# alex880317/LeGO-LOAM-SR

Measured on AMD Instinct MI355X. Metric: scans/sec (VLP-16 1800x16) at 1/2/4/8 GPUs; pose delta vs CPU ref, higher is better.
Workload: dtype fp32; 1 GPU; configs[1]: VLP-16 1800x16 projection + ground/cluster segmentation + curvature/feature extraction, labels/indices bit-exact vs CPU; lidar=VLP-16, rings=16, columns=1800, distinct_clouds_per_gpu=16, streams_per_gpu=3, parallelism=scan-sharded x1

## Files before the change

### lego-loam-sr_amd/csrc/llsr_fa.hip

```cpp
#include <cfloat>
#include <climits>

#include "llsr_device.h"
#include "llsr_imu.h"
#include "llsr_isort.h"
#include "llsr_libm.h"

namespace llsr {

using namespace llsr_libm;
constexpr double kPi = 3.14159265358979323846;

constexpr int kFaT = 256;
constexpr int kFaTile = 4 * kFaT - 12;

__device__ __forceinline__ float4 loam_point_rel(const DevCfg& c, float4 p, int i, int first, float start, float endo,
                                                 float diff, float* rel) {
  float o = -atan2f_(p.y, p.x);
  if (i <= first) {
    o = ori_branch1(o, start);
  } else {
    o = (float)(o + 2 * kPi);
    if ((double)o < (double)endo - kPi * 3 / 2) o = (float)(o + 2 * kPi);
    else if ((double)o > (double)endo + kPi / 2) o = (float)(o - 2 * kPi);
// ... 317 lines not shown
  const int l = lane_id();
  const unsigned long long lt = (1ull << l) - 1ull;
  int nsel = 0;
  for (int t0 = 0; t0 < nc; t0 += 64) {
    const int t = t0 + l;
    const bool valid = t < nc;
    const int ind = valid ? order(t) : 0;
    const int w = valid ? ind - ws : 0;
    const int r = valid ? wflag[w] : 0x80;
    bool alive = valid && (r & 0x80) == 0;
    const int lo = w - ((r >> 3) & 7), hi = w + (r & 7);
    unsigned long long sel = 0ull;
    unsigned long long m = __ballot(alive);
    while (m) {
      const int s = __ffsll((long long)m) - 1;
      const int slo = __builtin_amdgcn_readlane(lo, s), shi = __builtin_amdgcn_readlane(hi, s);
      sel |= 1ull << s;
      if (l > s && w >= slo && w <= shi) alive = false;
      if (l == s) alive = false;
      m = __ballot(alive);
    }
    if ((sel >> l) & 1ull) {
      wlab[w] = lab;
      outp[nsel + __popcll(sel & lt)] = ind;
      for (int q = lo; q <= hi; ++q) wflag[q] = (uint8_t)(wflag[q] | 0x80);
    }
    nsel += __popcll(sel);
    __builtin_amdgcn_fence(__ATOMIC_SEQ_CST, "wavefront");
    __builtin_amdgcn_wave_barrier();
  }
  return nsel;
}

__global__ __launch_bounds__(256, 5) void k_select_ring(DevCfg c, DevBufs d) {
  __shared__ uint64_t key[kRingMax];
  __shared__ uint32_t win_raw[2 * kWin / 4];
  uint8_t* wflag = reinterpret_cast<uint8_t*>(win_raw);
  int8_t* wlab = reinterpret_cast<int8_t*>(wflag + kWin);
  __shared__ uint16_t cfirst[kWin / 64 + 1];
  __shared__ uint16_t cpos[kRingMax];
  __shared__ uint16_t rstart[kRingMax + 1];
  __shared__ int tmp[8];
  __shared__ float red[6][4];
  __shared__ int s_cnt;
  const int i = blockIdx.x, b = blockIdx.y;
  const int H = c.H, HW = c.HW;
  const size_t base = (size_t)b * HW;
  const int tid = threadIdx.x, nt = blockDim.x;
  int* rc = d.ring_cnt + (size_t)b * 3 * H;
  const int sp = d.start_ring[b * H + i];
  const int ep = d.end_ring[b * H + i] - 1;
  if (sp >= ep) {
    if (tid == 0) { rc[i] = 0; rc[H + i] = 0; rc[2 * H + i] = 0; }
    return;
  }
  const float* curv = d.curv + base;
  const int ws = sp - 5 > 0 ? sp - 5 : 0;
  const int we = ep + 5 < HW - 1 ? ep + 5 : HW - 1;
  const int wn = we - ws + 1;
  if (c.dbg_phase <= -2) return;
  constexpr int kPer = (kWin + 255) / 256;
  float cvr[kPer];
  uint32_t cl[kPer];
  uint32_t pkm = 0, gdm = 0;
  {
    uint8_t pk[kPer], gd[kPer];
    int8_t lb[kPer];
#pragma unroll
    for (int u = 0; u < kPer; ++u) {
      const int t = tid + u * 256, pos = ws + t;
      cl[u] = 0;
      if (t < wn) {
        pk[u] = d.picked[base + pos];
        gd[u] = d.seg_ground[base + pos];
        lb[u] = d.clabel[base + pos];
        cl[u] = d.seg_col[base + pos];
        cvr[u] = curv[pos];
      }
    }
#pragma unroll
    for (int u = 0; u < kPer; ++u) {
      const int t = tid + u * 256;
      if (t < wn) {
        wlab[t] = lb[u];
        pkm |= (pk[u] != 0 ? 1u : 0u) << u;
        gdm |= (gd[u] != 0 ? 1u : 0u) << u;
        if ((t & 63) == 0) cfirst[t >> 6] = (uint16_t)cl[u];
      }
    }
  }
  if (tid == 0) s_cnt = 0;
  __syncthreads();
  if (c.dbg_phase <= -1) return;
  {
    uint64_t* gbits = reinterpret_cast<uint64_t*>(key);
    const int l = lane_id();
#pragma unroll
    for (int u = 0; u < kPer; ++u) {
      const int t = tid + u * 256;
      const int dn = __shfl_down((int)cl[u], 1, 64);
      const int nx = l < 63 ? dn : (t + 1 < wn ? (int)cfirst[(t + 1) >> 6] : 0);
      const bool stop = t + 1 >= wn || abs(nx - (int)cl[u]) > 10;
      const uint64_t m = __ballot(t < wn && stop);
      if (l == 0 && (t >> 6) <= (wn >> 6)) gbits[t >> 6] = m;
    }
    __syncthreads();
    const int nw = (wn >> 6) + 1;
#pragma unroll
    for (int u = 0; u < kPer; ++u) {
      const int t = tid + u * 256;
      if (t >= wn) break;
      const int k = t >> 6, sh = t & 63;
      uint64_t fw = gbits[k] >> sh;
      if (sh && k + 1 < nw) fw |= gbits[k + 1] << (64 - sh);
      const int f = fw ? min(5, __ffsll((long long)fw) - 1) : 5;
      int bk = 0;
      if (t > 0) {
        const int q = t - 1, kq = q >> 6, s2 = q & 63;
        uint64_t bw = gbits[kq] << (63 - s2);
        if (s2 < 63 && kq > 0) bw |= gbits[kq - 1] >> (s2 + 1);
        bk = min(min(5, t), bw ? (int)__clzll((long long)bw) : 64);
      }
      wflag[t] = (uint8_t)(f | (bk << 3) | (((gdm >> u) & 1u) << 6) | (((pkm >> u) & 1u) << 7));
    }
  }
  __syncthreads();
  const int nRng = ep - sp;
  const int ph = sp == 4 ? d.phantom[b] : 0;
  const bool ph_in = ph >= ws && ph - ws < wn;
  const float ph_curv = ph < 5 ? 0.0f : curv[ph];
  if (sp == 4 && !ph_in && tid == 0) atomicAdd(&d.counts[b * kCnt + C_PHOUT], 1);
  __shared__ BlockSortLds bsl;
  __shared__ int s_flag, s_exact;
  if (tid == 0) s_flag = 0;
  __syncthreads();
  if (sp == 4) {
#pragma unroll
    for (int u = 0; u < kPer; ++u) {
      const int p = ws + tid + u * 256;
      if (p >= 5 && p < ep && cvr[u] == 0.0f) s_flag = 1;
    }
  }
  auto curv_of = [&](int ind) { return ind < 5 ? 0.0f : curv[ind]; };
  auto exact_sort = [&]() {
    for (int t = tid; t < nRng; t += nt) {
      const int p = sp + t;
      const float v = p == 4 ? 0.0f : curv[p];
      const int ind = p == 4 ? ph : p;
      key[t] = ((uint64_t)__float_as_uint(v) << 32) | (uint32_t)ind;
    }
    block_introsort<256>(key, nRng, cpos, rstart, bsl, CurvLess{});
    if (tid == 0) {
      if (sp == 4) d.phantom[b] = (int)(uint32_t)key[0];
      atomicAdd(&d.counts[b * kCnt + C_EXACT], 1);
      s_exact = 1;
    }
    __syncthreads();
  };
  auto compact_sorted = [&](bool descending, auto elig) {
    const int l = lane_id();
    int cnt = 0;
    for (int c0 = 0; c0 < nRng; c0 += 64) {
      const int k = c0 + l;
      const int t = descending ? nRng - 1 - k : k;
      const bool e = k < nRng && elig((int)(uint32_t)key[t]);
      const unsigned long long m = __ballot(e);
      if (e) cpos[cnt + __popcll(m & ((1ull << l) - 1ull))] = (uint16_t)t;
      cnt += __popcll(m);
    }
    return cnt;
  };
  auto edge_elig = [&](int ind) {
    const int w = ind - ws;
    return w >= 0 && w < wn && (wflag[w] & 0xC0) == 0 && curv_of(ind) > c.edge_thr;
  };
  auto flat_elig = [&](int ind) {
    const int w = ind - ws;
    return w >= 0 && w < wn && (wflag[w] & 0xC0) == 0x40 && curv_of(ind) < c.surf_thr;
  };
  auto append = [&](bool edge) {
#pragma unroll
    for (int u = 0; u < kPer; ++u) {
      const int p = ws + tid + u * 256;
      const bool in = p >= sp && p < ep && (p != 4 || ph_in);
      const int ind = p == 4 ? ph : p;
      const float v = p == 4 ? 0.0f : cvr[u];
      const float ve = p == 4 ? ph_curv : cvr[u];
      const int w = in ? ind - ws : 0;
      const int fg = in ? (wflag[w] & 0xC0) : 0x80;
      const bool e = in && (edge ? (fg == 0 && ve > c.edge_thr) : (fg == 0x40 && ve < c.surf_thr));
      const unsigned long long m = __ballot(e);
      int wb = 0;
      if (lane_id() == 0 && m) wb = atomicAdd(&s_cnt, (int)__popcll(m));
      wb = __builtin_amdgcn_readlane(wb, 0);
      if (e) key[wb + __popcll(m & ((1ull << lane_id()) - 1ull))] = ((uint64_t)__float_as_uint(v) << 32) | (uint32_t)ind;
    }
  };
  auto ties = [&](int lo, int hi) {
    for (int t = lo + tid; t + 1 < hi; t += nt)
      if ((uint32_t)(key[t] >> 32) == (uint32_t)(key[t + 1] >> 32)) s_flag = 1;
    __syncthreads();
    return s_flag != 0;
  };
  if (tid == 0) s_exact = 0;
  __syncthreads();
  const bool epE = curv[ep] > c.edge_thr && (wflag[ep - ws] & 0x40) == 0;
  const int e0 = epE ? 1 : 0;
  append(true);
  __syncthreads();
  if (c.dbg_phase <= 0) return;
  int nE = s_cnt;
  int n2 = max(pow2_ceil(nE), 64);
  for (int t = nE + tid; t < n2; t += nt) key[t] = 0ull;
  __syncthreads();
  block4_sort<uint64_t>(key, n2);
  if (c.dbg_phase <= 1) return;
  if (ties(n2 - nE, n2)) {
    exact_sort();
    if (tid < 64) {
      const int cnt = compact_sorted(true, edge_elig);
      auto order = [&](int t) { return t < e0 ? ep : (int)(uint32_t)key[cpos[t - e0]]; };
      const int sel = greedy_wave(order, cnt + e0, ws, wflag, wlab, (int8_t)1, d.edge_tmp + base + sp);
      if (tid == 0) { rc[i] = sel; s_cnt = 0; }
    }
  } else if (tid < 64) {
    auto order = [&](int t) { return t < e0 ? ep : (int)(uint32_t)key[n2 - 1 - (t - e0)]; };
    const int cnt = greedy_wave(order, nE + e0, ws, wflag, wlab, (int8_t)1, d.edge_tmp + base + sp);
    if (tid == 0) { rc[i] = cnt; s_cnt = 0; }
  }
  __syncthreads();
  if (c.dbg_phase <= 2) return;
  const bool epF = curv[ep] < c.surf_thr && (wflag[ep - ws] & 0x40) != 0;
  if (s_exact) {
    if (tid < 64) {
      const int cnt = compact_sorted(false, flat_elig);
      auto order = [&](int t) { return t < cnt ? (int)(uint32_t)key[cpos[t]] : ep; };
      const int sel = greedy_wave(order, cnt + (epF ? 1 : 0), ws, wflag, wlab, (int8_t)-1, d.flat_tmp + base + sp);
      if (tid == 0) rc[H + i] = sel;
    }
  } else {
    append(false);
    __syncthreads();
    const int nF = s_cnt;
    n2 = max(pow2_ceil(nF), 64);
    for (int t = nF + tid; t < n2; t += nt) key[t] = ~0ull;
    __syncthreads();
    block4_sort<uint64_t>(key, n2);
    if (ties(0, nF)) {
      exact_sort();
      if (tid < 64) {
        const int cnt = compact_sorted(false, flat_elig);
        auto order = [&](int t) { return t < cnt ? (int)(uint32_t)key[cpos[t]] : ep; };
        const int sel = greedy_wave(order, cnt + (epF ? 1 : 0), ws, wflag, wlab, (int8_t)-1, d.flat_tmp + base + sp);
        if (tid == 0) rc[H + i] = sel;
      }
    } else if (tid < 64) {
      auto order = [&](int t) { return t < nF ? (int)(uint32_t)key[t] : ep; };
      const int cnt = greedy_wave(order, nF + (epF ? 1 : 0), ws, wflag, wlab, (int8_t)-1, d.flat_tmp + base + sp);
      if (tid == 0) rc[H + i] = cnt;
    }
  }
  __syncthreads();
  if (c.dbg_phase <= 3) return;
  for (int t = tid; t < wn; t += nt) {
    d.picked[base + ws + t] = (uint8_t)(wflag[t] >> 7);
    d.clabel[base + ws + t] = wlab[t];
  }
  const int n = ep - sp + 1;
  const int per = (n + nt - 1) / nt;
  const int k0 = min(tid * per, n), k1 = min(k0 + per, n);
  int mine = 0;
  for (int k = k0; k < k1; ++k) mine += wlab[sp + k - ws] <= 0;
  int L;
  int pos = block_excl_scan(mine, tmp, &L);
  for (int k = k0; k < k1; ++k)
    if (wlab[sp + k - ws] <= 0) cpos[pos++] = (uint16_t)k;
  __syncthreads();
  if (c.dbg_phase <= 4) return;
  const float4* lp = d.loam + base + sp;
  constexpr int kLp = kRingMax / 256;
  float4 lpr[kLp];
  float mn[3] = {FLT_MAX, FLT_MAX, FLT_MAX}, mx[3] = {-FLT_MAX, -FLT_MAX, -FLT_MAX};
#pragma unroll
  for (int u = 0; u < kLp; ++u)
    if (tid + u * 256 < L) lpr[u] = lp[cpos[tid + u * 256]];
#pragma unroll
  for (int u = 0; u < kLp; ++u) {
    if (tid + u * 256 >= L) continue;
    const float4 p = lpr[u];
    mn[0] = fminf(mn[0], p.x); mn[1] = fminf(mn[1], p.y); mn[2] = fminf(mn[2], p.z);
    mx[0] = fmaxf(mx[0], p.x); mx[1] = fmaxf(mx[1], p.y); mx[2] = fmaxf(mx[2], p.z);
  }
  for (int a = 0; a < 3; ++a) { mn[a] = wave_reduce_min(mn[a]); mx[a] = wave_reduce_max(mx[a]); }
  if (lane_id() == 0)
    for (int a = 0; a < 3; ++a) { red[a][tid >> 6] = mn[a]; red[3 + a][tid >> 6] = mx[a]; }
  __syncthreads();
  for (int a = 0; a < 3; ++a) {
    mn[a] = fminf(fminf(red[a][0], red[a][1]), fminf(red[a][2], red[a][3]));
    mx[a] = fmaxf(fmaxf(red[3 + a][0], red[3 + a][1]), fmaxf(red[3 + a][2], red[3 + a][3]));
  }
  const float inv = 1.0f / 0.2f;
  float4* out = d.lflat_tmp + base + sp;
  if (L == 0) {
    if (tid == 0) rc[2 * H + i] = 0;
    return;
  }
  const long long dx = (long long)((mx[0] - mn[0]) * inv) + 1, dy = (long long)((mx[1] - mn[1]) * inv) + 1,
                  dz = (long long)((mx[2] - mn[2]) * inv) + 1;
  if (dx * dy * dz > (long long)INT_MAX) {
    for (int t = tid; t < L; t += nt) out[t] = lp[cpos[t]];
    if (tid == 0) rc[2 * H + i] = L;
    return;
  }
  int minb[3], div[3];
  for (int a = 0; a < 3; ++a) {
    minb[a] = (int)floorf(mn[a] * inv);
    div[a] = (int)floorf(mx[a] * inv) - minb[a] + 1;
  }
  const int mul1 = div[0], mul2 = div[0] * div[1];
  uint32_t* vk = reinterpret_cast<uint32_t*>(key);
  uint32_t vkr[kLp];
#pragma unroll
  for (int u = 0; u < kLp; ++u) {
    const int t = tid + u * 256;
    vkr[u] = 0u;
    if (t >= L) continue;
    const float4 p = lpr[u];
    const int i0 = (int)(floorf(p.x * inv) - (float)minb[0]);
    const int i1 = (int)(floorf(p.y * inv) - (float)minb[1]);
    const int i2 = (int)(floorf(p.z * inv) - (float)minb[2]);
    vkr[u] = (uint32_t)(i0 + i1 * mul1 + i2 * mul2);
    vk[t] = vkr[u];
  }
  __syncthreads();
  __shared__ int scnt[kLp * 4 + 1];
  const int wv = tid >> 6, ln = lane_id();
  const unsigned long long ltm = (1ull << ln) - 1ull;
  int V;
  auto slot_scan = [&]() {
    __syncthreads();
    if (wv == 0) {
      const int v = ln < kLp * 4 ? scnt[ln] : 0;
      const int incl = wave_incl_scan_add(v);
      if (ln < kLp * 4) scnt[ln] = incl - v;
      if (ln == 63) scnt[kLp * 4] = incl;
    }
    __syncthreads();
  };
  auto sort_runs = [&]() {
    unsigned long long mR[kLp];
#pragma unroll
    for (int u = 0; u < kLp; ++u) {
      const int t = u * 256 + tid;
      mR[u] = __ballot(t < L && (t == 0 || vkr[u] != vk[t - 1]));
      if (ln == 0) scnt[u * 4 + wv] = (int)__popcll(mR[u]);
    }
    slot_scan();
    const int R = scnt[kLp * 4];
#pragma unroll
    for (int u = 0; u < kLp; ++u) {
      if (!((mR[u] >> ln) & 1ull)) continue;
      const int t = u * 256 + tid;
      const int ro = scnt[u * 4 + wv] + (int)__popcll(mR[u] & ltm);
      rstart[ro] = (uint16_t)t;
      key[ro] = ((uint64_t)vkr[u] << 32) | (uint32_t)ro;
    }
    if (tid == 0) rstart[R] = (uint16_t)L;
    const int R2 = max(pow2_ceil(R), 64);
    for (int t = R + tid; t < R2; t += nt) key[t] = ~0ull;
    __syncthreads();
    block4_sort<uint64_t>(key, R2);
    return R;
  };
  if (c.exact_vg) {
    if (c.dbg_phase <= 5) return;
    const int R = sort_runs();
    uint16_t* rrank = reinterpret_cast<uint16_t*>(win_raw);
    const unsigned long long lem = ltm | (1ull << ln);
    unsigned long long mH[kLp];
#pragma unroll
    for (int u = 0; u < kLp; ++u) {
      const int t = u * 256 + tid;
      mH[u] = __ballot(t < R && (t == 0 || (key[t] >> 32) != (key[t - 1] >> 32)));
      if (ln == 0) scnt[u * 4 + wv] = (int)__popcll(mH[u]);
    }
    slot_scan();
#pragma unroll
    for (int u = 0; u < kLp; ++u) {
      const int t = u * 256 + tid;
      if (t < R) rrank[(uint32_t)key[t]] = (uint16_t)(scnt[u * 4 + wv] + (int)__popcll(mH[u] & lem) - 1);
    }
    __syncthreads();
    uint32_t* gk = reinterpret_cast<uint32_t*>(d.ccl_a + base) + sp;
    uint16_t* gc = reinterpret_cast<uint16_t*>(d.ccl_b + base) + sp;
    for (int r = tid; r < R; r += nt) {
      const uint32_t rk = (uint32_t)rrank[r] << 11;
      const int qe = rstart[r + 1];
      for (int q = rstart[r]; q < qe; ++q) gk[q] = rk | (uint32_t)q;
    }
    for (int t = tid; t < L; t += nt) gc[t] = cpos[t];
    if (tid == 0) rc[2 * H + i] = -1 - L;
    return;
  } else {
    if (c.dbg_phase <= 5) return;
    const int R = sort_runs();
    if (c.dbg_phase <= 6) return;
    unsigned long long mH[kLp];
#pragma unroll
    for (int u = 0; u < kLp; ++u) {
      const int t = u * 256 + tid;
      const bool head = t < R && (t == 0 || (key[t] >> 32) != (key[t - 1] >> 32));
      mH[u] = __ballot(head);
      if (ln == 0) scnt[u * 4 + wv] = (int)__popcll(mH[u]);
    }
    slot_scan();
    V = scnt[kLp * 4];
#pragma unroll
    for (int u = 0; u < kLp; ++u) {
      const int t = u * 256 + tid;
      if (!((mH[u] >> ln) & 1ull)) continue;
      const uint32_t vid = (uint32_t)(key[t] >> 32);
      float sx = 0.f, sy = 0.f, sz = 0.f, si = 0.f;
      int cntp = 0;
      for (int e = t; e < R && (uint32_t)(key[e] >> 32) == vid; ++e) {
        const int run = (int)(uint32_t)key[e];
        const int qe = rstart[run + 1];
        for (int q = rstart[run]; q < qe; q += 2) {
          const bool two = q + 1 < qe;
          const float4 p0 = lp[cpos[q]];
          const float4 p1 = two ? lp[cpos[q + 1]] : make_float4(0.f, 0.f, 0.f, 0.f);
          sx += p0.x; sy += p0.y; sz += p0.z; si += p0.w;
          ++cntp;
          if (two) {
            sx += p1.x; sy += p1.y; sz += p1.z; si += p1.w;
            ++cntp;
          }
        }
      }
      const float nn = (float)cntp;
      const int vo = scnt[u * 4 + wv] + (int)__popcll(mH[u] & ltm);
      out[vo] = make_float4(sx / nn, sy / nn, sz / nn, si / nn);
    }
  }
  if (tid == 0) rc[2 * H + i] = V;
}

__device__ __forceinline__ uint32_t* vox_keys(const DevCfg& c, const DevBufs& d, int slot) {
  return reinterpret_cast<uint32_t*>(d.ccl_a + (size_t)(slot / c.H) * c.HW) + d.start_ring[slot];
}

__global__ __launch_bounds__(256, 8) void k_vox_top(DevCfg c, DevBufs d, VoxRanges vr) {
// ... 643 lines not shown
```

### lego-loam-sr_amd/csrc/llsr_capi.hip

```cpp
#include <hip/hip_runtime.h>

#include <algorithm>
#include <climits>
#include <cmath>
#include <cstdio>
#include <cstdlib>
#include <cstring>
#include <memory>
#include <new>
#include <vector>

#include "llsr_handle.h"
#include "llsr_isort.h"
#include "llsr_libm.h"

namespace llsr {
template <bool kRanked> __global__ void k_project(DevCfg, const float4*, const int64_t*, DevBufs, const uint32_t*);
__global__ void k_row_bins(DevCfg, const float4*, const int64_t*, uint32_t*);
__global__ void k_gather_column(DevCfg, const float4*, const int64_t*, DevBufs);
__global__ void k_project_fused(DevCfg, const float4*, const int64_t*, DevBufs);
__global__ void k_ground_add(DevCfg, DevBufs);
__global__ void k_ground_elev_ransac(DevCfg, DevBufs);
template <bool kLds> __global__ void k_label(DevCfg, DevBufs);
__global__ void k_segment(DevCfg, const float4*, const int64_t*, DevBufs);
void launch_fa_points(const DevCfg&, const DevBufs&, int, hipStream_t);
void launch_fa_points_imu(const DevCfg&, const DevBufs&, const ImuDev&, int, hipStream_t);
__global__ void k_select_ring(DevCfg, DevBufs);
__global__ void k_vox_top(DevCfg, DevBufs, VoxRanges);
__global__ void k_vox_leaf(DevCfg, DevBufs, VoxRanges);
__global__ void k_vox_sum(DevCfg, DevBufs);
__global__ void k_debug_exact_sort(const float*, int, int*);
__global__ void k_debug_half_passed(const float*, int, uint8_t*);
__global__ void k_fa_concat(DevCfg, DevBufs);
__global__ void k_dbscan_adj(DevCfg, DevBufs, const float4* __restrict__);
__global__ void k_vis_clouds(DevCfg, DevBufs, int, float4*, int*);
template <int kDbL> __global__ void k_dbscan_merge(DevCfg, DevBufs);

__global__ void k_init_counts(int* counts, int B, int* vox_count) {
  const int b = blockIdx.x * blockDim.x + threadIdx.x;
  if (b < kVoxSub) vox_count[b * kVoxCntStride] = 0;
  if (b >= B) return;
  int* c = counts + b * kCnt;
  for (int k = 0; k < kCnt; ++k) c[k] = 0;
  c[C_FIRST] = INT_MAX;
  c[C_LAST] = -1;
}
}

using namespace llsr;

namespace {
const char* kKernelNames[] = {"init",          "k_project",    "k_gather_column", "k_ground_add",
                              "k_ground_elev_ransac", "k_label", "k_segment",      "k_fa_points",
                              "k_select_ring", "k_vox_pcl", "k_fa_concat", "k_dbscan_adj", "k_dbscan_merge",
                              "k_row_bins"};
static_assert(sizeof kKernelNames / sizeof *kKernelNames == kNumKernels, "one name per timed kernel");
}

static int row_bin_bound(const DevCfg& c) {
  const int top = trunc_i32((double)(1.57079637050628662109375f + c.ip_angBottom) / (0.335 * (M_PI / 180.0)));
  return top < 0 ? top : top + 1;
}

static int fused_lds(const DevCfg& c) { return c.HW * (int)sizeof(int); }
// ... 513 lines not shown
    if (ranks[t] >= (1u << 21)) return LLSR_EINVAL;
  if (n == 0) return LLSR_OK;
  std::vector<uint32_t> key(n);
  for (int32_t t = 0; t < n; ++t) key[t] = (ranks[t] << 11) | (uint32_t)t;
  const int head[4] = {0, 0, -1 - n, 0};
  int device = 0;
  llsr_host::DevMem dk, dh, di;
  if (hipGetDevice(&device) != hipSuccess || llsr_host::alloc(dk, sizeof(uint32_t) * n) != hipSuccess ||
      llsr_host::alloc(dh, sizeof head) != hipSuccess ||
      llsr_host::alloc(di, sizeof(int2) * kBsList * kVoxSub + kVoxCntBytes) != hipSuccess)
    return LLSR_ENODEV;
  int2* items = static_cast<int2*>(di.get());
  if (hipMemcpy(dk, key.data(), sizeof(uint32_t) * n, hipMemcpyHostToDevice) != hipSuccess ||
      hipMemcpy(dh, head, sizeof head, hipMemcpyHostToDevice) != hipSuccess ||
      hipMemset(items + kBsList * kVoxSub, 0, kVoxCntBytes) != hipSuccess)
    return LLSR_EIO;
  DevCfg c{};
  c.H = 1;
  c.W = c.HW = n;
  c.dbg_phase = 102;
  DevBufs d{};
  d.ccl_a = static_cast<int*>(dk.get());
  d.ring_cnt = static_cast<int*>(dh.get());
  d.start_ring = d.ring_cnt + 3;
  const VoxRanges vr{items, reinterpret_cast<int*>(items + kBsList * kVoxSub), kBsList};
  launch_vox_pcl(c, d, vr, vox_leaf_waves(device), 1, nullptr);
  if (hipGetLastError() != hipSuccess || hipDeviceSynchronize() != hipSuccess ||
      hipMemcpy(key.data(), dk, sizeof(uint32_t) * n, hipMemcpyDeviceToHost) != hipSuccess)
    return LLSR_EIO;
  for (int32_t t = 0; t < n; ++t) out[t] = (int32_t)(key[t] & 0x7ffu);
  return LLSR_OK;
}

extern "C" int32_t llsr_debug_dbscan_merge(const uint32_t* adj, const int32_t* M, int32_t n, int32_t kDbL,
                                           int32_t* cluster, int32_t* sharp, int32_t* n_sharp) {
  if (!adj || !M || !cluster || !sharp || !n_sharp || n < 1 || n > 1024 || (kDbL != 1024 && kDbL != 2048))
    return LLSR_EINVAL;
  for (int32_t k = 0; k < n; ++k)
    if (M[k] < 0 || M[k] > kDbL) return LLSR_EINVAL;
  const size_t HW = kAdjCap, nadj = (size_t)n * kAdjCap * kAdjWords;
  std::vector<int> cnt((size_t)n * kCnt, 0), pos((size_t)n * HW);
  for (int32_t k = 0; k < n; ++k) {
    cnt[(size_t)k * kCnt + C_M] = M[k];
    for (size_t a = 0; a < HW; ++a) pos[k * HW + a] = (int)a;
  }
  llsr_host::DevMem dadj, dcnt, dpos, dcl, dsh;
  if (llsr_host::alloc(dadj, sizeof(uint32_t) * nadj) != hipSuccess ||
      llsr_host::alloc(dcnt, sizeof(int) * cnt.size()) != hipSuccess ||
      llsr_host::alloc(dpos, sizeof(int) * n * HW) != hipSuccess ||
      llsr_host::alloc(dcl, sizeof(int) * n * HW) != hipSuccess ||
      llsr_host::alloc(dsh, sizeof(int) * n * HW) != hipSuccess)
    return LLSR_ENODEV;
  if (hipMemcpy(dadj, adj, sizeof(uint32_t) * nadj, hipMemcpyHostToDevice) != hipSuccess ||
      hipMemcpy(dcnt, cnt.data(), sizeof(int) * cnt.size(), hipMemcpyHostToDevice) != hipSuccess ||
      hipMemcpy(dpos, pos.data(), sizeof(int) * n * HW, hipMemcpyHostToDevice) != hipSuccess ||
      hipMemset(dcl, 0xff, sizeof(int) * n * HW) != hipSuccess ||
      hipMemset(dsh, 0xff, sizeof(int) * n * HW) != hipSuccess)
    return LLSR_EIO;
  DevCfg c{};
  c.HW = (int)HW;
  DevBufs d{};
  d.counts = static_cast<int*>(dcnt.get());
  d.db_adj = static_cast<uint32_t*>(dadj.get());
  d.less_sharp = static_cast<int*>(dpos.get());
  d.cluster = static_cast<int*>(dcl.get());
  d.sharp = static_cast<int*>(dsh.get());
// ... 13 lines not shown
  if (n == 0) return LLSR_OK;
  llsr_host::DevMem dv, dout;
  if (llsr_host::alloc(dv, sizeof(float) * 3 * (size_t)n) != hipSuccess ||
      llsr_host::alloc(dout, 3 * (size_t)n) != hipSuccess)
    return LLSR_ENODEV;
  if (hipMemcpy(dv, yxs, sizeof(float) * 3 * (size_t)n, hipMemcpyHostToDevice) != hipSuccess) return LLSR_EIO;
  k_debug_half_passed<<<(n + 255) / 256, 256>>>((const float*)dv.get(), n, (uint8_t*)dout.get());
  if (hipGetLastError() != hipSuccess || hipDeviceSynchronize() != hipSuccess ||
      hipMemcpy(out, dout, 3 * (size_t)n, hipMemcpyDeviceToHost) != hipSuccess)
    return LLSR_EIO;
  return LLSR_OK;
}

extern "C" float llsr_debug_exact_sort_ms(const float* vals, int32_t n, int32_t reps) {
  if (!vals || n < 1 || n > 2048 || reps < 1) return -1.f;
  llsr_host::DevMem dv, di;
  llsr_host::Event e0, e1;
  float ms = -1.f;
  if (llsr_host::alloc(dv, sizeof(float) * n) == hipSuccess && llsr_host::alloc(di, sizeof(int) * n) == hipSuccess &&
      llsr_host::create(e0) == hipSuccess && llsr_host::create(e1) == hipSuccess &&
      hipMemcpy(dv, vals, sizeof(float) * n, hipMemcpyHostToDevice) == hipSuccess) {
    k_debug_exact_sort<<<1, 256>>>((const float*)dv.get(), n, (int*)di.get());
    (void)hipEventRecord(e0, nullptr);
    for (int r = 0; r < reps; ++r) k_debug_exact_sort<<<1, 256>>>((const float*)dv.get(), n, (int*)di.get());
    (void)hipEventRecord(e1, nullptr);
    if (hipEventSynchronize(e1) == hipSuccess && hipEventElapsedTime(&ms, e0, e1) == hipSuccess) ms /= reps;
  }
  return ms;
}

static void restore_selection(llsr_handle* h, int B, hipStream_t s) {
  const DevCfg& c = h->dc;
  launch_fa_points(c, h->d, B, s);
  k_select_ring<<<dim3(c.H, B), 256, 0, s>>>(c, h->d);
  if (c.exact_vg) {
    (void)hipMemsetAsync(h->vox.count, 0, kVoxCntBytes, s);
    launch_vox_pcl(c, h->d, h->vox, h->vox_waves, B, s);
  }
  (void)hipStreamSynchronize(s);
}

extern "C" float llsr_debug_phase_ms(llsr_handle* h, int32_t k, int32_t phase, int32_t reps) {
  if (!h || h->last_B < 1 || reps < 1) return -1.f;
  if (hipSetDevice(h->device) != hipSuccess) return -1.f;
  hipStream_t s = h->stream;
  DevCfg c = h->dc;
  c.dbg_phase = phase;
  const int B = h->last_B;
  hipEvent_t e0 = h->ev[0][0], e1 = h->ev[0][1];
  if (sync_last(h) != LLSR_OK) return -1.f;
  if (k == 9) {
    float tot = 0.f;
    for (int r = 0; r < reps; ++r) {
      launch_fa_points(h->dc, h->d, B, s);
      k_select_ring<<<dim3(c.H, B), 256, 0, s>>>(h->dc, h->d);
      (void)hipMemsetAsync(h->vox.count, 0, kVoxCntBytes, s);
      (void)hipEventRecord(e0, s);
      launch_vox_pcl(c, h->d, h->vox, h->vox_waves, B, s);
      (void)hipEventRecord(e1, s);
      float ms = 0.f;
      if (hipEventSynchronize(e1) != hipSuccess || hipEventElapsedTime(&ms, e0, e1) != hipSuccess) return -1.f;
      tot += ms;
    }
    restore_selection(h, B, s);
    return tot / reps;
  }
// ... 150 lines not shown
```

### lego-loam-sr_amd/csrc/llsr_device.h

```cpp
#pragma once
#include <hip/hip_runtime.h>
#include <stdint.h>

#include "../../include/llsr.h"
#include "llsr_libm.h"

namespace llsr {

enum : int {
  C_NPTS = 0,
  C_FIRST = 1,
  C_LAST = 2,
  C_S = 3,
  C_O = 4,
  C_K = 5,
  C_INL = 6,
  C_RIT = 7,
  C_M = 8,
  C_SHARP = 9,
  C_F = 10,
  C_L = 11,
  C_HALF = 12,
  C_EXACT = 13,
  C_PHOUT = 14,
  kCnt = 16
};

struct DevCfg {
  int H, W, HW;
  float ip_resX, ip_resY, ip_angBottom;
  float segThr, sinX, cosX, sinY, cosY;
  int use_kitti, gsi, pointNum, lineNum;
  float scan_period, edge_thr, surf_thr;
  float fa_resY, sinResX, RatioXY, RatioZ, DBFr;
  float gnd_cos[3];
  int ccl_lds;
  int lbl_band;
  int exact_vg;
  int dbg_phase;
  int use_vlp32c;
};

constexpr int kBinWords = 16;

struct DevBufs {
  int* counts;
  float* orient;
  int* cell_pt;
  float* range;
  float4* full;
  int8_t* ground;
  int* label;
  float4* near_pts;
  int* shuf;
  int* ccl_a;
  unsigned long long* ccl_b;
  int* start_ring;
// ... 221 lines not shown
```

Before: 370,400 scans/s.

## Bound per-ring loops by live chunk count, skip empty sorts, ballot-compact labels

```diff
diff --git a/lego-loam-sr_amd/csrc/llsr_fa.hip b/lego-loam-sr_amd/csrc/llsr_fa.hip
--- a/lego-loam-sr_amd/csrc/llsr_fa.hip
+++ b/lego-loam-sr_amd/csrc/llsr_fa.hip
@@ -381,7 +381,6 @@
   __shared__ uint16_t cfirst[kWin / 64 + 1];
   __shared__ uint16_t cpos[kRingMax];
   __shared__ uint16_t rstart[kRingMax + 1];
-  __shared__ int tmp[8];
   __shared__ float red[6][4];
   __shared__ int s_cnt;
   const int i = blockIdx.x, b = blockIdx.y;
@@ -401,16 +400,17 @@
   const int wn = we - ws + 1;
   if (c.dbg_phase <= -2) return;
   constexpr int kPer = (kWin + 255) / 256;
+  const int nwp = __builtin_amdgcn_readfirstlane((wn + 255) >> 8);
   float cvr[kPer];
-  uint32_t cl[kPer];
+  uint32_t cl[kPer] = {};
   uint32_t pkm = 0, gdm = 0;
   {
     uint8_t pk[kPer], gd[kPer];
     int8_t lb[kPer];
 #pragma unroll
     for (int u = 0; u < kPer; ++u) {
+      if (u >= nwp) continue;
       const int t = tid + u * 256, pos = ws + t;
-      cl[u] = 0;
       if (t < wn) {
         pk[u] = d.picked[base + pos];
         gd[u] = d.seg_ground[base + pos];
@@ -421,6 +421,7 @@
     }
 #pragma unroll
     for (int u = 0; u < kPer; ++u) {
+      if (u >= nwp) continue;
       const int t = tid + u * 256;
       if (t < wn) {
         wlab[t] = lb[u];
@@ -436,8 +437,10 @@
   {
     uint64_t* gbits = reinterpret_cast<uint64_t*>(key);
     const int l = lane_id();
+    const int nws = __builtin_amdgcn_readfirstlane((wn >> 8) + 1);
 #pragma unroll
     for (int u = 0; u < kPer; ++u) {
+      if (u >= nws) continue;
       const int t = tid + u * 256;
       const int dn = __shfl_down((int)cl[u], 1, 64);
       const int nx = l < 63 ? dn : (t + 1 < wn ? (int)cfirst[(t + 1) >> 6] : 0);
@@ -449,8 +452,9 @@
     const int nw = (wn >> 6) + 1;
 #pragma unroll
     for (int u = 0; u < kPer; ++u) {
+      if (u >= nwp) continue;
       const int t = tid + u * 256;
-      if (t >= wn) break;
+      if (t >= wn) continue;
       const int k = t >> 6, sh = t & 63;
       uint64_t fw = gbits[k] >> sh;
       if (sh && k + 1 < nw) fw |= gbits[k + 1] << (64 - sh);
@@ -478,6 +482,7 @@
   if (sp == 4) {
 #pragma unroll
     for (int u = 0; u < kPer; ++u) {
+      if (u >= nwp) continue;
       const int p = ws + tid + u * 256;
       if (p >= 5 && p < ep && cvr[u] == 0.0f) s_flag = 1;
     }
@@ -522,6 +527,7 @@
   auto append = [&](bool edge) {
 #pragma unroll
     for (int u = 0; u < kPer; ++u) {
+      if (u >= nwp) continue;
       const int p = ws + tid + u * 256;
       const bool in = p >= sp && p < ep && (p != 4 || ph_in);
       const int ind = p == 4 ? ph : p;
@@ -551,12 +557,16 @@
   __syncthreads();
   if (c.dbg_phase <= 0) return;
   int nE = s_cnt;
-  int n2 = max(pow2_ceil(nE), 64);
-  for (int t = nE + tid; t < n2; t += nt) key[t] = 0ull;
-  __syncthreads();
-  block4_sort<uint64_t>(key, n2);
+  const bool noE = nE == 0 && s_flag == 0;
+  int n2 = 0;
+  if (!noE) {
+    n2 = max(pow2_ceil(nE), 64);
+    for (int t = nE + tid; t < n2; t += nt) key[t] = 0ull;
+    __syncthreads();
+    block4_sort<uint64_t>(key, n2);
+  }
   if (c.dbg_phase <= 1) return;
-  if (ties(n2 - nE, n2)) {
+  if (!noE && ties(n2 - nE, n2)) {
     exact_sort();
     if (tid < 64) {
       const int cnt = compact_sorted(true, edge_elig);
@@ -583,11 +593,15 @@
     append(false);
     __syncthreads();
     const int nF = s_cnt;
-    n2 = max(pow2_ceil(nF), 64);
-    for (int t = nF + tid; t < n2; t += nt) key[t] = ~0ull;
-    __syncthreads();
-    block4_sort<uint64_t>(key, n2);
-    if (ties(0, nF)) {
+    bool tie = false;
+    if (nF != 0) {
+      n2 = max(pow2_ceil(nF), 64);
+      for (int t = nF + tid; t < n2; t += nt) key[t] = ~0ull;
+      __syncthreads();
+      block4_sort<uint64_t>(key, n2);
+      tie = ties(0, nF);
+    }
+    if (tie) {
       exact_sort();
       if (tid < 64) {
         const int cnt = compact_sorted(false, flat_elig);
@@ -607,26 +621,54 @@
     d.picked[base + ws + t] = (uint8_t)(wflag[t] >> 7);
     d.clabel[base + ws + t] = wlab[t];
   }
+  constexpr int kLp = kRingMax / 256;
+  __shared__ int scnt[kLp * 4 + 1];
+  const int wv = tid >> 6, ln = lane_id();
+  const unsigned long long ltm = (1ull << ln) - 1ull;
+  auto slot_scan = [&](int ns) {
+    __syncthreads();
+    if (wv == 0) {
+      const int v = ln < ns * 4 ? scnt[ln] : 0;
+      const int incl = wave_incl_scan_add(v);
+      if (ln < ns * 4) scnt[ln] = incl - v;
+      if (ln == 63) scnt[kLp * 4] = incl;
+    }
+    __syncthreads();
+  };
   const int n = ep - sp + 1;
-  const int per = (n + nt - 1) / nt;
-  const int k0 = min(tid * per, n), k1 = min(k0 + per, n);
-  int mine = 0;
-  for (int k = k0; k < k1; ++k) mine += wlab[sp + k - ws] <= 0;
-  int L;
-  int pos = block_excl_scan(mine, tmp, &L);
-  for (int k = k0; k < k1; ++k)
-    if (wlab[sp + k - ws] <= 0) cpos[pos++] = (uint16_t)k;
+  const int nsn = __builtin_amdgcn_readfirstlane((n + 255) >> 8);
+  {
+    const int8_t* rl = wlab + (sp - ws);
+    unsigned long long mC[kLp];
+#pragma unroll
+    for (int u = 0; u < kLp; ++u) {
+      if (u >= nsn) continue;
+      const int k = u * 256 + tid;
+      mC[u] = __ballot(k < n && rl[k] <= 0);
+      if (ln == 0) scnt[u * 4 + wv] = (int)__popcll(mC[u]);
+    }
+    slot_scan(nsn);
+#pragma unroll
+    for (int u = 0; u < kLp; ++u) {
+      if (u >= nsn) continue;
+      if ((mC[u] >> ln) & 1ull) cpos[scnt[u * 4 + wv] + (int)__popcll(mC[u] & ltm)] = (uint16_t)(u * 256 + tid);
+    }
+  }
+  const int L = scnt[kLp * 4];
   __syncthreads();
   if (c.dbg_phase <= 4) return;
   const float4* lp = d.loam + base + sp;
-  constexpr int kLp = kRingMax / 256;
+  const int nlp = __builtin_amdgcn_readfirstlane((L + 255) >> 8);
   float4 lpr[kLp];
   float mn[3] = {FLT_MAX, FLT_MAX, FLT_MAX}, mx[3] = {-FLT_MAX, -FLT_MAX, -FLT_MAX};
 #pragma unroll
-  for (int u = 0; u < kLp; ++u)
+  for (int u = 0; u < kLp; ++u) {
+    if (u >= nlp) continue;
     if (tid + u * 256 < L) lpr[u] = lp[cpos[tid + u * 256]];
+  }
 #pragma unroll
   for (int u = 0; u < kLp; ++u) {
+    if (u >= nlp) continue;
     if (tid + u * 256 >= L) continue;
     const float4 p = lpr[u];
     mn[0] = fminf(mn[0], p.x); mn[1] = fminf(mn[1], p.y); mn[2] = fminf(mn[2], p.z);
@@ -663,6 +705,7 @@
   uint32_t vkr[kLp];
 #pragma unroll
   for (int u = 0; u < kLp; ++u) {
+    if (u >= nlp) continue;
     const int t = tid + u * 256;
     vkr[u] = 0u;
     if (t >= L) continue;
@@ -674,32 +717,23 @@
     vk[t] = vkr[u];
   }
   __syncthreads();
-  __shared__ int scnt[kLp * 4 + 1];
-  const int wv = tid >> 6, ln = lane_id();
-  const unsigned long long ltm = (1ull << ln) - 1ull;
   int V;
-  auto slot_scan = [&]() {
-    __syncthreads();
-    if (wv == 0) {
-      const int v = ln < kLp * 4 ? scnt[ln] : 0;
-      const int incl = wave_incl_scan_add(v);
-      if (ln < kLp * 4) scnt[ln] = incl - v;
-      if (ln == 63) scnt[kLp * 4] = incl;
-    }
-    __syncthreads();
-  };
+  int crun[kLp];
   auto sort_runs = [&]() {
     unsigned long long mR[kLp];
 #pragma unroll
     for (int u = 0; u < kLp; ++u) {
+      if (u >= nlp) continue;
       const int t = u * 256 + tid;
       mR[u] = __ballot(t < L && (t == 0 || vkr[u] != vk[t - 1]));
       if (ln == 0) scnt[u * 4 + wv] = (int)__popcll(mR[u]);
     }
-    slot_scan();
+    slot_scan(nlp);
     const int R = scnt[kLp * 4];
 #pragma unroll
     for (int u = 0; u < kLp; ++u) {
+      if (u >= nlp) continue;
+      crun[u] = scnt[u * 4 + wv] + (int)__popcll(mR[u] & (ltm | (1ull << ln))) - 1;
       if (!((mR[u] >> ln) & 1ull)) continue;
       const int t = u * 256 + tid;
       const int ro = scnt[u * 4 + wv] + (int)__popcll(mR[u] & ltm);
@@ -716,30 +750,36 @@
   if (c.exact_vg) {
     if (c.dbg_phase <= 5) return;
     const int R = sort_runs();
+    if (c.dbg_phase <= 6) return;
     uint16_t* rrank = reinterpret_cast<uint16_t*>(win_raw);
     const unsigned long long lem = ltm | (1ull << ln);
     unsigned long long mH[kLp];
 #pragma unroll
     for (int u = 0; u < kLp; ++u) {
+      if (u >= nlp) continue;
       const int t = u * 256 + tid;
       mH[u] = __ballot(t < R && (t == 0 || (key[t] >> 32) != (key[t - 1] >> 32)));
       if (ln == 0) scnt[u * 4 + wv] = (int)__popcll(mH[u]);
     }
-    slot_scan();
+    slot_scan(nlp);
 #pragma unroll
     for (int u = 0; u < kLp; ++u) {
+      if (u >= nlp) continue;
       const int t = u * 256 + tid;
       if (t < R) rrank[(uint32_t)key[t]] = (uint16_t)(scnt[u * 4 + wv] + (int)__popcll(mH[u] & lem) - 1);
     }
     __syncthreads();
     uint32_t* gk = reinterpret_cast<uint32_t*>(d.ccl_a + base) + sp;
     uint16_t* gc = reinterpret_cast<uint16_t*>(d.ccl_b + base) + sp;
-    for (int r = tid; r < R; r += nt) {
-      const uint32_t rk = (uint32_t)rrank[r] << 11;
-      const int qe = rstart[r + 1];
-      for (int q = rstart[r]; q < qe; ++q) gk[q] = rk | (uint32_t)q;
-    }
-    for (int t = tid; t < L; t += nt) gc[t] = cpos[t];
+#pragma unroll
+    for (int u = 0; u < kLp; ++u) {
+      if (u >= nlp) continue;
+      const int t = u * 256 + tid;
+      if (t < L) {
+        gk[t] = ((uint32_t)rrank[crun[u]] << 11) | (uint32_t)t;
+        gc[t] = cpos[t];
+      }
+    }
     if (tid == 0) rc[2 * H + i] = -1 - L;
     return;
   } else {
@@ -749,15 +789,17 @@
     unsigned long long mH[kLp];
 #pragma unroll
     for (int u = 0; u < kLp; ++u) {
+      if (u >= nlp) continue;
       const int t = u * 256 + tid;
       const bool head = t < R && (t == 0 || (key[t] >> 32) != (key[t - 1] >> 32));
       mH[u] = __ballot(head);
       if (ln == 0) scnt[u * 4 + wv] = (int)__popcll(mH[u]);
     }
-    slot_scan();
+    slot_scan(nlp);
     V = scnt[kLp * 4];
 #pragma unroll
     for (int u = 0; u < kLp; ++u) {
+      if (u >= nlp) continue;
       const int t = u * 256 + tid;
       if (!((mH[u] >> ln) & 1ull)) continue;
       const uint32_t vid = (uint32_t)(key[t] >> 32);
```

Result: no change. 371,600 scans/s, median of 6 (+0.3%).

## Replace voxel run sort with bitmap row ranking in exact voxel-grid key path

Applied to the files above, without the earlier changes.

```diff
diff --git a/lego-loam-sr_amd/csrc/llsr_capi.hip b/lego-loam-sr_amd/csrc/llsr_capi.hip
--- a/lego-loam-sr_amd/csrc/llsr_capi.hip
+++ b/lego-loam-sr_amd/csrc/llsr_capi.hip
@@ -30,6 +30,7 @@
 __global__ void k_vox_leaf(DevCfg, DevBufs, VoxRanges);
 __global__ void k_vox_sum(DevCfg, DevBufs);
 __global__ void k_debug_exact_sort(const float*, int, int*);
+__global__ void k_debug_vox_keys(const float4*, int, int, uint32_t*, int*);
 __global__ void k_debug_half_passed(const float*, int, uint8_t*);
 __global__ void k_fa_concat(DevCfg, DevBufs);
 __global__ void k_dbscan_adj(DevCfg, DevBufs, const float4* __restrict__);
@@ -609,6 +610,36 @@
   return LLSR_OK;
 }
 
+extern "C" int32_t llsr_debug_vox_keys(const float* points, int32_t L, int32_t force_runs, uint32_t* keys_out,
+                                       int32_t* path_out) {
+  if (!points || !keys_out || !path_out || L < 1 || L > 2048) return LLSR_EINVAL;
+  llsr_host::DevMem dp, dk, dq;
+  if (llsr_host::alloc(dp, sizeof(float4) * L) != hipSuccess || llsr_host::alloc(dk, sizeof(uint32_t) * L) != hipSuccess ||
+      llsr_host::alloc(dq, sizeof(int)) != hipSuccess)
+    return LLSR_ENODEV;
+  if (hipMemcpy(dp, points, sizeof(float4) * L, hipMemcpyHostToDevice) != hipSuccess ||
+      hipMemset(dk, 0, sizeof(uint32_t) * L) != hipSuccess)
+    return LLSR_EIO;
+  k_debug_vox_keys<<<1, 256>>>((const float4*)dp.get(), L, force_runs, (uint32_t*)dk.get(), (int*)dq.get());
+  int path = 0;
+  if (hipGetLastError() != hipSuccess || hipDeviceSynchronize() != hipSuccess ||
+      hipMemcpy(keys_out, dk, sizeof(uint32_t) * L, hipMemcpyDeviceToHost) != hipSuccess ||
+      hipMemcpy(&path, dq, sizeof(int), hipMemcpyDeviceToHost) != hipSuccess)
+    return LLSR_EIO;
+  *path_out = path;
+  return LLSR_OK;
+}
+
+extern "C" int32_t llsr_debug_vox_runs(llsr_handle* h, int32_t* out) {
+  if (!h || !out) return LLSR_EINVAL;
+  int32_t rc = sync_last(h);
+  if (rc) return rc;
+  std::vector<int> cnt((size_t)h->last_B * kCnt);
+  HIP_OK(h, hipMemcpy(cnt.data(), h->d.counts, cnt.size() * sizeof(int), hipMemcpyDeviceToHost));
+  for (int b = 0; b < h->last_B; ++b) out[b] = cnt[(size_t)b * kCnt + C_VOXRUNS];
+  return LLSR_OK;
+}
+
 extern "C" int32_t llsr_debug_dbscan_merge(const uint32_t* adj, const int32_t* M, int32_t n, int32_t kDbL,
                                            int32_t* cluster, int32_t* sharp, int32_t* n_sharp) {
   if (!adj || !M || !cluster || !sharp || !n_sharp || n < 1 || n > 1024 || (kDbL != 1024 && kDbL != 2048))
@@ -688,6 +719,7 @@
 static void restore_selection(llsr_handle* h, int B, hipStream_t s) {
   const DevCfg& c = h->dc;
   launch_fa_points(c, h->d, B, s);
+  (void)hipMemset2DAsync(h->d.counts + C_VOXRUNS, sizeof(int) * kCnt, 0, sizeof(int), B, s);
   k_select_ring<<<dim3(c.H, B), 256, 0, s>>>(c, h->d);
   if (c.exact_vg) {
     (void)hipMemsetAsync(h->vox.count, 0, kVoxCntBytes, s);
diff --git a/lego-loam-sr_amd/csrc/llsr_device.h b/lego-loam-sr_amd/csrc/llsr_device.h
--- a/lego-loam-sr_amd/csrc/llsr_device.h
+++ b/lego-loam-sr_amd/csrc/llsr_device.h
@@ -23,6 +23,7 @@
   C_HALF = 12,
   C_EXACT = 13,
   C_PHOUT = 14,
+  C_VOXRUNS = 15,
   kCnt = 16
 };
 
diff --git a/lego-loam-sr_amd/csrc/llsr_fa.hip b/lego-loam-sr_amd/csrc/llsr_fa.hip
--- a/lego-loam-sr_amd/csrc/llsr_fa.hip
+++ b/lego-loam-sr_amd/csrc/llsr_fa.hip
@@ -373,6 +373,206 @@
   return nsel;
 }
 
+constexpr int kRingLp = kRingMax / 256;
+constexpr int kVoxRowBits = kRingMax * 64;
+constexpr int kVoxI0Bits = 10;
+
+struct VoxKeyLds {
+  uint64_t* key;
+  uint16_t* rstart;
+  uint16_t* rrank;
+  int* scnt;
+  int* tmp;
+};
+
+__device__ __forceinline__ void vox_bounds(const float4 (&lpr)[kRingLp], int L, float (*red)[4], float (&mn)[3],
+                                           float (&mx)[3]) {
+  const int tid = threadIdx.x;
+  for (int a = 0; a < 3; ++a) { mn[a] = FLT_MAX; mx[a] = -FLT_MAX; }
+#pragma unroll
+  for (int u = 0; u < kRingLp; ++u) {
+    if (tid + u * 256 >= L) continue;
+    const float4 p = lpr[u];
+    mn[0] = fminf(mn[0], p.x); mn[1] = fminf(mn[1], p.y); mn[2] = fminf(mn[2], p.z);
+    mx[0] = fmaxf(mx[0], p.x); mx[1] = fmaxf(mx[1], p.y); mx[2] = fmaxf(mx[2], p.z);
+  }
+  for (int a = 0; a < 3; ++a) { mn[a] = wave_reduce_min(mn[a]); mx[a] = wave_reduce_max(mx[a]); }
+  if (lane_id() == 0)
+    for (int a = 0; a < 3; ++a) { red[a][tid >> 6] = mn[a]; red[3 + a][tid >> 6] = mx[a]; }
+  __syncthreads();
+  for (int a = 0; a < 3; ++a) {
+    mn[a] = fminf(fminf(red[a][0], red[a][1]), fminf(red[a][2], red[a][3]));
+    mx[a] = fmaxf(fmaxf(red[3 + a][0], red[3 + a][1]), fmaxf(red[3 + a][2], red[3 + a][3]));
+  }
+}
+__device__ __forceinline__ bool vox_grid(const float (&mn)[3], const float (&mx)[3], int (&minb)[3], int (&div)[3]) {
+  const float inv = 1.0f / 0.2f;
+  const long long dx = (long long)((mx[0] - mn[0]) * inv) + 1, dy = (long long)((mx[1] - mn[1]) * inv) + 1,
+                  dz = (long long)((mx[2] - mn[2]) * inv) + 1;
+  if (dx * dy * dz > (long long)INT_MAX) return false;
+  for (int a = 0; a < 3; ++a) {
+    minb[a] = (int)floorf(mn[a] * inv);
+    div[a] = (int)floorf(mx[a] * inv) - minb[a] + 1;
+  }
+  return true;
+}
+__device__ __forceinline__ void vox_cell(const float4 p, const int (&minb)[3], int& i0, int& i1, int& i2) {
+  const float inv = 1.0f / 0.2f;
+  i0 = (int)(floorf(p.x * inv) - (float)minb[0]);
+  i1 = (int)(floorf(p.y * inv) - (float)minb[1]);
+  i2 = (int)(floorf(p.z * inv) - (float)minb[2]);
+}
+__device__ __forceinline__ void vox_ids(const float4 (&lpr)[kRingLp], int L, const int (&minb)[3], const int (&div)[3],
+                                        uint32_t (&vkr)[kRingLp], uint64_t* key) {
+  const int mul1 = div[0], mul2 = div[0] * div[1];
+  uint32_t* vk = reinterpret_cast<uint32_t*>(key);
+#pragma unroll
+  for (int u = 0; u < kRingLp; ++u) {
+    const int t = threadIdx.x + u * 256;
+    vkr[u] = 0u;
+    if (t >= L) continue;
+    int i0, i1, i2;
+    vox_cell(lpr[u], minb, i0, i1, i2);
+    vkr[u] = (uint32_t)(i0 + i1 * mul1 + i2 * mul2);
+    vk[t] = vkr[u];
+  }
+  __syncthreads();
+}
+__device__ __forceinline__ void vox_slot_scan(int* scnt) {
+  __syncthreads();
+  if (threadIdx.x < 64) {
+    const int ln = threadIdx.x;
+    const int v = ln < kRingLp * 4 ? scnt[ln] : 0;
+    const int incl = wave_incl_scan_add(v);
+    if (ln < kRingLp * 4) scnt[ln] = incl - v;
+    if (ln == 63) scnt[kRingLp * 4] = incl;
+  }
+  __syncthreads();
+}
+__device__ __forceinline__ int vox_sort_runs(const uint32_t (&vkr)[kRingLp], int L, const VoxKeyLds& s) {
+  const int tid = threadIdx.x, wv = tid >> 6, ln = lane_id();
+  const unsigned long long ltm = (1ull << ln) - 1ull;
+  const uint32_t* vk = reinterpret_cast<const uint32_t*>(s.key);
+  unsigned long long mR[kRingLp];
+#pragma unroll
+  for (int u = 0; u < kRingLp; ++u) {
+    const int t = u * 256 + tid;
+    mR[u] = __ballot(t < L && (t == 0 || vkr[u] != vk[t - 1]));
+    if (ln == 0) s.scnt[u * 4 + wv] = (int)__popcll(mR[u]);
+  }
+  vox_slot_scan(s.scnt);
+  const int R = s.scnt[kRingLp * 4];
+#pragma unroll
+  for (int u = 0; u < kRingLp; ++u) {
+    if (!((mR[u] >> ln) & 1ull)) continue;
+    const int t = u * 256 + tid;
+    const int ro = s.scnt[u * 4 + wv] + (int)__popcll(mR[u] & ltm);
+    s.rstart[ro] = (uint16_t)t;
+    s.key[ro] = ((uint64_t)vkr[u] << 32) | (uint32_t)ro;
+  }
+  if (tid == 0) s.rstart[R] = (uint16_t)L;
+  const int R2 = max(pow2_ceil(R), 64);
+  for (int t = R + tid; t < R2; t += 256) s.key[t] = ~0ull;
+  __syncthreads();
+  block4_sort<uint64_t>(s.key, R2);
+  return R;
+}
+
+__device__ __forceinline__ int vox_pcl_keys(const float4 (&lpr)[kRingLp], int L, const int (&minb)[3],
+                                            const int (&div)[3], bool force_runs, const VoxKeyLds& s, uint32_t* gk) {
+  const int tid = threadIdx.x, wv = tid >> 6, ln = lane_id();
+  const long long rows = (long long)div[1] * div[2];
+  if (!force_runs && div[0] <= (1 << kVoxI0Bits) && rows <= kVoxRowBits) {
+    const int nW = ((int)rows + 63) >> 6;
+    for (int w = tid; w < nW; w += 256) s.key[w] = 0ull;
+    uint32_t row[kRingLp], i0r[kRingLp];
+#pragma unroll
+    for (int u = 0; u < kRingLp; ++u) {
+      row[u] = i0r[u] = 0u;
+      if (tid + u * 256 >= L) continue;
+      int i0, i1, i2;
+      vox_cell(lpr[u], minb, i0, i1, i2);
+      row[u] = min((uint32_t)(i1 + i2 * div[1]), (uint32_t)rows - 1u);
+      i0r[u] = min((uint32_t)i0, (1u << kVoxI0Bits) - 1u);
+    }
+    __syncthreads();
+#pragma unroll
+    for (int u = 0; u < kRingLp; ++u)
+      if (tid + u * 256 < L)
+        atomicOr(reinterpret_cast<uint32_t*>(s.key) + (row[u] >> 5), 1u << (row[u] & 31u));
+    __syncthreads();
+    const int per = (nW + 255) >> 8;
+    const int w0 = min(tid * per, nW), w1 = min(w0 + per, nW);
+    int cnt = 0;
+    for (int w = w0; w < w1; ++w) cnt += (int)__popcll(s.key[w]);
+    const int incl = wave_incl_scan_add(cnt);
+    if (ln == 63) s.tmp[wv] = incl;
+    __syncthreads();
+    int pre = incl - cnt;
+    for (int k = 0; k < wv; ++k) pre += s.tmp[k];
+    for (int w = w0; w < w1; ++w) {
+      s.rstart[w] = (uint16_t)pre;
+      pre += (int)__popcll(s.key[w]);
+    }
+    __syncthreads();
+#pragma unroll
+    for (int u = 0; u < kRingLp; ++u) {
+      const int t = tid + u * 256;
+      if (t >= L) continue;
+      const uint64_t wd = s.key[row[u] >> 6];
+      const uint32_t rr = (uint32_t)s.rstart[row[u] >> 6] + (uint32_t)__popcll(wd & ((1ull << (row[u] & 63u)) - 1ull));
+      gk[t] = (((rr << kVoxI0Bits) | i0r[u]) << 11) | (uint32_t)t;
+    }
+    return 0;
+  }
+  uint32_t vkr[kRingLp];
+  vox_ids(lpr, L, minb, div, vkr, s.key);
+  const int R = vox_sort_runs(vkr, L, s);
+  const unsigned long long lem = ((1ull << ln) - 1ull) | (1ull << ln);
+  unsigned long long mH[kRingLp];
+#pragma unroll
+  for (int u = 0; u < kRingLp; ++u) {
+    const int t = u * 256 + tid;
+    mH[u] = __ballot(t < R && (t == 0 || (s.key[t] >> 32) != (s.key[t - 1] >> 32)));
+    if (ln == 0) s.scnt[u * 4 + wv] = (int)__popcll(mH[u]);
+  }
+  vox_slot_scan(s.scnt);
+#pragma unroll
+  for (int u = 0; u < kRingLp; ++u) {
+    const int t = u * 256 + tid;
+    if (t < R) s.rrank[(uint32_t)s.key[t]] = (uint16_t)(s.scnt[u * 4 + wv] + (int)__popcll(mH[u] & lem) - 1);
+  }
+  __syncthreads();
+  for (int r = tid; r < R; r += 256) {
+    const uint32_t rk = (uint32_t)s.rrank[r] << 11;
+    const int qe = s.rstart[r + 1];
+    for (int q = s.rstart[r]; q < qe; ++q) gk[q] = rk | (uint32_t)q;
+  }
+  return 1;
+}
+
+__global__ __launch_bounds__(256) void k_debug_vox_keys(const float4* pts, int L, int force_runs, uint32_t* keys,
+                                                        int* path) {
+  __shared__ uint64_t key[kRingMax];
+  __shared__ uint16_t rstart[kRingMax + 1], rrank[kRingMax];
+  __shared__ int scnt[kRingLp * 4 + 1], tmp[8];
+  __shared__ float red[6][4];
+  const int tid = threadIdx.x;
+  float4 lpr[kRingLp];
+#pragma unroll
+  for (int u = 0; u < kRingLp; ++u)
+    if (tid + u * 256 < L) lpr[u] = pts[tid + u * 256];
+  float mn[3], mx[3];
+  vox_bounds(lpr, L, red, mn, mx);
+  int minb[3], div[3];
+  if (!vox_grid(mn, mx, minb, div)) {
+    if (tid == 0) *path = -1;
+    return;
+  }
+  const int p = vox_pcl_keys(lpr, L, minb, div, force_runs != 0, VoxKeyLds{key, rstart, rrank, scnt, tmp}, keys);
+  if (tid == 0) *path = p;
+}
+
 __global__ __launch_bounds__(256, 5) void k_select_ring(DevCfg c, DevBufs d) {
   __shared__ uint64_t key[kRingMax];
   __shared__ uint32_t win_raw[2 * kWin / 4];
@@ -619,132 +819,45 @@
   __syncthreads();
   if (c.dbg_phase <= 4) return;
   const float4* lp = d.loam + base + sp;
-  constexpr int kLp = kRingMax / 256;
+  constexpr int kLp = kRingLp;
   float4 lpr[kLp];
-  float mn[3] = {FLT_MAX, FLT_MAX, FLT_MAX}, mx[3] = {-FLT_MAX, -FLT_MAX, -FLT_MAX};
 #pragma unroll
   for (int u = 0; u < kLp; ++u)
     if (tid + u * 256 < L) lpr[u] = lp[cpos[tid + u * 256]];
-#pragma unroll
-  for (int u = 0; u < kLp; ++u) {
-    if (tid + u * 256 >= L) continue;
-    const float4 p = lpr[u];
-    mn[0] = fminf(mn[0], p.x); mn[1] = fminf(mn[1], p.y); mn[2] = fminf(mn[2], p.z);
-    mx[0] = fmaxf(mx[0], p.x); mx[1] = fmaxf(mx[1], p.y); mx[2] = fmaxf(mx[2], p.z);
-  }
-  for (int a = 0; a < 3; ++a) { mn[a] = wave_reduce_min(mn[a]); mx[a] = wave_reduce_max(mx[a]); }
-  if (lane_id() == 0)
-    for (int a = 0; a < 3; ++a) { red[a][tid >> 6] = mn[a]; red[3 + a][tid >> 6] = mx[a]; }
-  __syncthreads();
-  for (int a = 0; a < 3; ++a) {
-    mn[a] = fminf(fminf(red[a][0], red[a][1]), fminf(red[a][2], red[a][3]));
-    mx[a] = fmaxf(fmaxf(red[3 + a][0], red[3 + a][1]), fmaxf(red[3 + a][2], red[3 + a][3]));
-  }
-  const float inv = 1.0f / 0.2f;
+  float mn[3], mx[3];
+  vox_bounds(lpr, L, red, mn, mx);
   float4* out = d.lflat_tmp + base + sp;
   if (L == 0) {
     if (tid == 0) rc[2 * H + i] = 0;
     return;
   }
-  const long long dx = (long long)((mx[0] - mn[0]) * inv) + 1, dy = (long long)((mx[1] - mn[1]) * inv) + 1,
-                  dz = (long long)((mx[2] - mn[2]) * inv) + 1;
-  if (dx * dy * dz > (long long)INT_MAX) {
+  int minb[3], div[3];
+  if (!vox_grid(mn, mx, minb, div)) {
     for (int t = tid; t < L; t += nt) out[t] = lp[cpos[t]];
     if (tid == 0) rc[2 * H + i] = L;
     return;
   }
-  int minb[3], div[3];
-  for (int a = 0; a < 3; ++a) {
-    minb[a] = (int)floorf(mn[a] * inv);
-    div[a] = (int)floorf(mx[a] * inv) - minb[a] + 1;
-  }
-  const int mul1 = div[0], mul2 = div[0] * div[1];
-  uint32_t* vk = reinterpret_cast<uint32_t*>(key);
-  uint32_t vkr[kLp];
-#pragma unroll
-  for (int u = 0; u < kLp; ++u) {
-    const int t = tid + u * 256;
-    vkr[u] = 0u;
-    if (t >= L) continue;
-    const float4 p = lpr[u];
-    const int i0 = (int)(floorf(p.x * inv) - (float)minb[0]);
-    const int i1 = (int)(floorf(p.y * inv) - (float)minb[1]);
-    const int i2 = (int)(floorf(p.z * inv) - (float)minb[2]);
-    vkr[u] = (uint32_t)(i0 + i1 * mul1 + i2 * mul2);
-    vk[t] = vkr[u];
-  }
-  __syncthreads();
   __shared__ int scnt[kLp * 4 + 1];
+  const VoxKeyLds vl{key, rstart, reinterpret_cast<uint16_t*>(win_raw), scnt, tmp};
   const int wv = tid >> 6, ln = lane_id();
   const unsigned long long ltm = (1ull << ln) - 1ull;
   int V;
-  auto slot_scan = [&]() {
-    __syncthreads();
-    if (wv == 0) {
-      const int v = ln < kLp * 4 ? scnt[ln] : 0;
-      const int incl = wave_incl_scan_add(v);
-      if (ln < kLp * 4) scnt[ln] = incl - v;
-      if (ln == 63) scnt[kLp * 4] = incl;
-    }
-    __syncthreads();
-  };
-  auto sort_runs = [&]() {
-    unsigned long long mR[kLp];
-#pragma unroll
-    for (int u = 0; u < kLp; ++u) {
-      const int t = u * 256 + tid;
-      mR[u] = __ballot(t < L && (t == 0 || vkr[u] != vk[t - 1]));
-      if (ln == 0) scnt[u * 4 + wv] = (int)__popcll(mR[u]);
-    }
-    slot_scan();
-    const int R = scnt[kLp * 4];
-#pragma unroll
-    for (int u = 0; u < kLp; ++u) {
-      if (!((mR[u] >> ln) & 1ull)) continue;
-      const int t = u * 256 + tid;
-      const int ro = scnt[u * 4 + wv] + (int)__popcll(mR[u] & ltm);
-      rstart[ro] = (uint16_t)t;
-      key[ro] = ((uint64_t)vkr[u] << 32) | (uint32_t)ro;
-    }
-    if (tid == 0) rstart[R] = (uint16_t)L;
-    const int R2 = max(pow2_ceil(R), 64);
-    for (int t = R + tid; t < R2; t += nt) key[t] = ~0ull;
-    __syncthreads();
-    block4_sort<uint64_t>(key, R2);
-    return R;
-  };
   if (c.exact_vg) {
     if (c.dbg_phase <= 5) return;
-    const int R = sort_runs();
-    uint16_t* rrank = reinterpret_cast<uint16_t*>(win_raw);
-    const unsigned long long lem = ltm | (1ull << ln);
-    unsigned long long mH[kLp];
-#pragma unroll
-    for (int u = 0; u < kLp; ++u) {
-      const int t = u * 256 + tid;
-      mH[u] = __ballot(t < R && (t == 0 || (key[t] >> 32) != (key[t - 1] >> 32)));
-      if (ln == 0) scnt[u * 4 + wv] = (int)__popcll(mH[u]);
-    }
-    slot_scan();
-#pragma unroll
-    for (int u = 0; u < kLp; ++u) {
-      const int t = u * 256 + tid;
-      if (t < R) rrank[(uint32_t)key[t]] = (uint16_t)(scnt[u * 4 + wv] + (int)__popcll(mH[u] & lem) - 1);
-    }
-    __syncthreads();
     uint32_t* gk = reinterpret_cast<uint32_t*>(d.ccl_a + base) + sp;
     uint16_t* gc = reinterpret_cast<uint16_t*>(d.ccl_b + base) + sp;
-    for (int r = tid; r < R; r += nt) {
-      const uint32_t rk = (uint32_t)rrank[r] << 11;
-      const int qe = rstart[r + 1];
-      for (int q = rstart[r]; q < qe; ++q) gk[q] = rk | (uint32_t)q;
-    }
+    const int path = vox_pcl_keys(lpr, L, minb, div, false, vl, gk);
     for (int t = tid; t < L; t += nt) gc[t] = cpos[t];
-    if (tid == 0) rc[2 * H + i] = -1 - L;
+    if (tid == 0) {
+      rc[2 * H + i] = -1 - L;
+      if (path) atomicAdd(&d.counts[b * kCnt + C_VOXRUNS], 1);
+    }
     return;
   } else {
+    uint32_t vkr[kLp];
+    vox_ids(lpr, L, minb, div, vkr, key);
     if (c.dbg_phase <= 5) return;
-    const int R = sort_runs();
+    const int R = vox_sort_runs(vkr, L, vl);
     if (c.dbg_phase <= 6) return;
     unsigned long long mH[kLp];
 #pragma unroll
@@ -754,7 +867,7 @@
       mH[u] = __ballot(head);
       if (ln == 0) scnt[u * 4 + wv] = (int)__popcll(mH[u]);
     }
-    slot_scan();
+    vox_slot_scan(scnt);
     V = scnt[kLp * 4];
 #pragma unroll
     for (int u = 0; u < kLp; ++u) {
```

After: 368,300 scans/s before, 384,800 scans/s after (median of 6 runs). 4.5% higher.
